# haampie/Homogenization.jl

Measured on AMD Instinct MI355X. Metric: fine-DOF updates/sec per V-cycle (3D Tet64), higher is better.
Workload: dtype f64; 1 GPU; 3D Tet64 checkerboard, 32^3 unit cubes x 6 tets, refinements=5 (BASELINE config 3); cells=196608, nf=6545, levels=6, smoothing_steps=3, smoothing_steps_coarse=2, coarse_solver=device CG, Chebyshev(4)-of-Jacobi preconditioner, rtol 1e-13, spare_vector_bytes=10294394880, lazy_top_form=2

## Files before the change

homogenization.jl_amd/csrc/hmg_context.cpp:

```cpp
#include "../../include/hmg.h"
#include "hmg_objects.hpp"

#include <algorithm>

namespace hmg {

std::recursive_mutex &lifetime_mutex()
{
    static std::recursive_mutex m;
    return m;
}

std::atomic<int64_t> &device_allocs()
{
    static std::atomic<int64_t> n{0};
    return n;
}

namespace {

void vec_pool_trim(hmg_ctx *c)
{
    LifetimeLock lock(lifetime_mutex());
    if (c->vec_pool.empty()) return;
// ... 206 lines not shown
}

int64_t hmg_ctx_counter(hmg_ctx *ctx, const char *name)
{
    if (!ctx || !name) return -1;
    const std::string n(name);
    if (n == "wave_launches") return ctx->wave_launches;
    if (n == "slab2_launches") return ctx->slab2_launches;
    if (n == "rows_launches") return ctx->rows_launches;
    if (n == "small_launches") return ctx->small_launches;
    if (n == "comm_calls") return ctx->comm_calls;
    if (n == "device_allocs") return device_allocs().load();
    if (n == "spare_bytes") return ctx->spare_bytes;
    if (n == "fcg_bytes") return ctx->fcg_bytes;
    if (n == "lazy_top_form") return ctx->last_top_form;
    if (n == "comm_nranks") return ctx->comm ? ctx->comm_nranks : 0;
    return -1;
}

int hmg_ctx_release_memory(hmg_ctx *ctx)
{
    HMG_TRY
    need(ctx != nullptr, "null ctx");
    vec_pool_trim(ctx);
    HMG_END
}

int hmg_ctx_set_option(hmg_ctx *ctx, const char *name, int64_t value)
{
    HMG_TRY
    need(ctx && name, "null argument");
    std::string n(name);
    static const std::pair<const char *, bool hmg_ctx::*> flags[] = {
        {"coarse_probe", &hmg_ctx::coarse_probe}, {"fuse_cg", &hmg_ctx::fuse_cg_default}, {"fold_x", &hmg_ctx::fold_x},
        {"swap_rp", &hmg_ctx::swap_rp}, {"fold_prolong", &hmg_ctx::fold_prolong}, {"zero_entry", &hmg_ctx::zero_entry},
        {"fold_restrict", &hmg_ctx::fold_restrict}, {"lazy_dead", &hmg_ctx::lazy_dead}, {"fold_faces", &hmg_ctx::fold_faces},
        {"lean_post", &hmg_ctx::lean_post}, {"lazy_post", &hmg_ctx::lazy_post}, {"prolong_in_image", &hmg_ctx::prolong_in_image},
        {"comm_rehearsal", &hmg_ctx::comm_rehearsal}};
    for (const auto &f : flags)
        if (n == f.first) {
            ctx->*f.second = value != 0;
            return 0;
        }
    if (n == "apply_threads")
        ctx->L.apply_threads = (int)value;
    else if (n == "apply_wg512")
        ctx->L.apply_wg512 = value != 0;
    else if (n == "apply_pack")
        ctx->L.apply_pack = value != 0;
    else if (n == "apply_small")
        ctx->L.apply_small = value != 0;
// ... 172 lines not shown
```

homogenization.jl_amd/csrc/hmg_device.hpp:

```cpp
#pragma once
#include <hip/hip_runtime.h>

#include <cstdint>

namespace hmg {

constexpr int TABLE_PAD = 3 * 1024;

__host__ __device__ inline int rows_slot(int m, int i, int j, int nei, int off_int, int &cls)
{
    if (j == 0) {
        cls = i == 0 ? 4 : i == m ? 5 : 1;
        return i == 0 ? 0 : i == m ? 1 : 3 + i - 1;
    }
    if (i == 0) {
        cls = j == m ? 6 : 2;
        return j == m ? 2 : 3 + nei + j - 1;
    }
    if (i + j == m) {
        cls = 3;
        return 3 + 2 * nei + j - 1;
    }
    cls = 0;
    return off_int + (j - 1) * (m - 1) - (((j - 1) * j) >> 1) + i - 1;
// ... 79 lines not shown
    int nclasses;
    double wc_lambda;
    double *blockpart;
    SlabTables slab;
};

struct ApplyArgs {
    double alpha, lambda;
    const double *x;
    const double *x2;
    double *xout;
    double *xacc;
    int a_num, a_den;
    const double *x3;
    int c_num, c_den;
    const double *xcoarse;
    int64_t ldc;
    const double *src;
    double *out;
    double *rcoarse;
    int64_t ldrc;
    const double *scal;
    int s_num, s_den;
    double *blockpart;
    const uint8_t *mult;
    int flags;
    int64_t ncells_prefix;
    int64_t out_ld;
    const int32_t *cell_list;
    int64_t ncell_list;
    int64_t nwork;
    const int32_t *cell_class;
// ... 28 lines not shown
    int apply_wave;
    int64_t wave_grid;
    int64_t *n_wave_launches;
    int apply_slab2;
    int64_t *n_slab2_launches;
    int64_t slab2_grid;
    int restrict_slab2;
    int slab2_force;
    int64_t *n_rows_launches;
};

void launch_apply(const Launch &L, const LevelDev &lv, const MeshDev &mesh, double alpha, double lambda,
                  const double *x, const double *src, double *out, int use_mask);
size_t apply_lds_bytes(const LevelDev &lv);
bool apply_restricts(const Launch &L, const LevelDev &lv);
void launch_apply_fused_kernel(const Launch &L, const LevelDev &lv, const MeshDev &mesh, ApplyArgs a);
void launch_apply_fused_reduce(const Launch &L, const MeshDev &mesh, int slot_pap, int slot_rr);
void launch_apply_args(const Launch &L, const LevelDev &lv, const MeshDev &mesh, ApplyArgs a);
bool apply_wave_ok(const Launch &L, const LevelDev &lv, const MeshDev &mesh, const ApplyArgs &a, bool fused);
void launch_apply_wave(const Launch &L, const LevelDev &lv, const MeshDev &mesh, const ApplyArgs &a, bool fused);
bool apply_slab2_ok(const Launch &L, const LevelDev &lv, const MeshDev &mesh, const ApplyArgs &a);
void launch_apply_slab2(const Launch &L, const LevelDev &lv, const MeshDev &mesh, const ApplyArgs &a, bool fused);
void launch_apply_rows(const Launch &L, const LevelDev &lv, const MeshDev &mesh, const ApplyArgs &a, bool fused, bool wd);
void launch_prolong_add_wide(const Launch &L, const LevelDev &fine, const LevelDev &coarse, int64_t ncells, const double *xc,
                             double *xf);
int64_t launch_norm2_unique_wide(const Launch &L, const LevelDev &lv, const MeshDev &mesh, const double *x);
bool apply_small_ok(const Launch &L, const LevelDev &lv, const MeshDev &mesh, const ApplyArgs &a, bool fused);
void launch_apply_small(const Launch &L, const LevelDev &lv, const MeshDev &mesh, const ApplyArgs &a, bool fused);
void launch_weight_cache(const Launch &L, const LevelDev &lv, const double *coef_rep, int nclasses, double lambda, double *wcache);

// ... 76 lines not shown
```

homogenization.jl_amd/csrc/hmg_kernels.hip:

```cpp
#include "hmg_device.hpp"
#include "hmg_stencil.hpp"

#include <cstdio>
#include <stdexcept>
#include <string>

namespace hmg {

__global__ void __launch_bounds__(256) k_finalize(const double *__restrict__ partials, int n, double *scal, int slot)
{
    __shared__ double red[4];
    double v = 0.0;
    for (int i = threadIdx.x; i < n; i += 256) v += partials[i];
    double s = block_sum(v, red);
    if (threadIdx.x == 0) scal[slot] = s;
}

#ifdef HMG_PHASE_TIMING
#define HMG_STAMP(i)                                                                     \
    do {    \
        if (a.blockpart && !a.cell_list && tid == 0)                                     \
            a.blockpart[2 * (size_t)a.nwork + 8 * cell + (i)] = (double)wall_clock64(); \
    } while (0)
#define HMG_SLAB_T0() const long long _t0 = wall_clock64(); long long _tl = _t0; double _ph[5] = {0, 0, 0, 0, 0}
// ... 174 lines not shown
            if (wave == NW - 1) {
                const int cbase = (1 + lv.nface + lv.nedge) * NDIR;
                for (int idx = cbase + lane; idx < lv.ncls * NDIR; idx += 64) {
                    double w = 0.0;
#pragma unroll
                    for (int t = 0; t < NTERM; ++t) w += lv.ctab[(size_t)idx * NTERM + t] * sc7[t];
                    W[idx - cbase] = w;
                }
            }
        }
        if (FUSED) {
#pragma unroll
            for (int q = 0; q < 4; ++q) mq[q] = a.mult ? __builtin_amdgcn_readfirstlane(mqr[q]) : 0x01010101u;
        }
    };
    constexpr bool rows_late = WC && LF == 2;
    constexpr bool WEARLY = false;
    if (EARLY && !rows_late) issue_rows();
    if (WEARLY) issue_words();
    const double *xc = a.x + cell * lv.ld;
    double rr = 0.0, pap = 0.0;
    {
        const double *x2c = FUSED && a.x2 ? a.x2 + cell * lv.ld : nullptr;
        double *xoc = FUSED && a.xout ? a.xout + cell * lv.ld : nullptr;
        double *xac = FUSED && a.xacc ? a.xacc + cell * lv.ld : nullptr;
        const double *x3c = FUSED && a.x3 ? a.x3 + cell * lv.ld : nullptr;
        const double beta = x2c ? a.scal[a.s_num] / a.scal[a.s_den] : 0.0;
        const double ax = xac || x3c ? a.scal[a.a_num] / a.scal[a.a_den] : 0.0;
        const double c2 = x3c ? a.scal[a.c_num] / a.scal[a.c_den] : 0.0;
        const double *ccol = FUSED && !RS && a.xcoarse ? a.xcoarse + cell * a.ldc : nullptr;
        constexpr bool cgather = FUSED && CG;
        double *cs = xs + nf + lv.lds_g1;
        double cval = 0.0;
        if (ccol && !cgather) {
            if (tid < lv.nf_coarse) cval = ccol[tid];
            for (int q = tid + NT; q < lv.nf_coarse; q += NT) cs[q] = ccol[q];
        }
        auto prolong = [&](double v, uint32_t w) {
            const uint32_t pa = w & 0xffffu, pb = w >> 16;
            if (pa == pb) return v + cs[pa];
            v += 0.5 * cs[pa];
            return v + 0.5 * cs[pb];
        };
        if (cgather && ccol) {
            constexpr int NC = 2;
            double cv2[NC];
            int cl2[NC];
#pragma unroll
            for (int q = 0; q < NC; ++q) {
                const int c = tid + q * NT;
                if (c < lv.nf_coarse) {
                    cv2[q] = ccol[c];
                    cl2[q] = lv.clpos[c];
                }
            }
            double xv[SPT];
            uint64_t pw[SPT];
#pragma unroll
            for (int q = 0; q < SPT; ++q) {
                const int t = tid + q * NT;
                if (t < nf) {
                    xv[q] = xc[t];
                    pw[q] = lv.par64[t];
                }
            }
            if (EARLY) finish_tables();
#pragma unroll
            for (int q = 0; q < NC; ++q)
                if (tid + q * NT < lv.nf_coarse) xs[cl2[q]] = cv2[q];
// ... 63 lines not shown
                }
            }
            if (EARLY && rows_late) issue_rows();
            if (EARLY) finish_tables();
#pragma unroll
            for (int q = 0; q < SPT; ++q) {
                const int t = tid + q * NT;
                if (t < nf) {
                    const double v = axpy1(beta, x2v[q], xv[q]);
                    if (LF == 2 && xoc) xoc[t] = v;
                    rr += v * v;
                    xs[lp[q]] = v;
                }
            }
        }
        constexpr int HB = FUSED ? (SPT + 1) / 2 : SPT;
        const bool xzero = FUSED && (RS || RB == 0) && (a.flags & 128);
        if (!light && !light2 && !(cgather && ccol)) {
#pragma unroll
        for (int q0 = 0; q0 < SPT; q0 += HB) {
            double xv[HB], x2v[HB], xav[HB];
            int lp[HB];
            uint32_t pw[HB];
#pragma unroll
            for (int q = 0; q < HB; ++q) {
                const int t = tid + (q0 + q) * NT;
                if (q0 + q < SPT && t < nf) {
                    xv[q] = xzero ? 0.0 : xc[t];
                    x2v[q] = x2c ? x2c[t] : 0.0;
                    xav[q] = xac ? xac[t] : x3c ? x3c[t] : 0.0;
                    lp[q] = lv.lpos[t];
                    if (FUSED && !cgather) pw[q] = ccol ? lv.par32[t] : 0u;
                }
            }
            if (EARLY && q0 == 0) finish_tables();
            if (FUSED && q0 == 0 && ccol && !cgather) {
                if (tid < lv.nf_coarse) cs[tid] = cval;
                __syncthreads();
            }
#pragma unroll
            for (int q = 0; q < HB; ++q) {
                const int t = tid + (q0 + q) * NT;
                if (q0 + q < SPT && t < nf) {
                    double v = xv[q];
                    if (FUSED) {
                        if (!cgather && ccol) v = prolong(v, pw[q]);
                        if (xac) xac[t] = axpy1(ax, x2v[q], xav[q]);
                        if (x3c) {
                            const double t1 = axpy1(ax, x2v[q], v);
                            const double p2 = axpy1(beta, x2v[q], xav[q]);
                            v = axpy1(c2, p2, t1);
                        } else if (x2c)
                            v = axpy1(beta, x2v[q], v);
                        if (xoc) xoc[t] = v;
                        if (!RS) rr += v * v;
                    }
                    xs[lp[q]] = v;
                }
            }
        }
        }
        for (int t = tid + SPT * NT; t < nf; t += NT) {
            double v = xzero ? 0.0 : xc[t];
            if (FUSED) {
                const double pv = x2c ? x2c[t] : 0.0;
                if (!cgather && ccol) v = prolong(v, lv.par32[t]);
                if (xac) xac[t] = axpy1(ax, pv, xac[t]);
                if (x3c) {
                    const double t1 = axpy1(ax, pv, v);
                    const double p2 = axpy1(beta, pv, x3c[t]);
                    v = axpy1(c2, p2, t1);
                } else if (x2c)
                    v = axpy1(beta, pv, v);
                if (xoc) xoc[t] = v;
                rr += v * v;
            }
            xs[lv.lpos[t]] = v;
        }
    }

    HMG_STAMP(1);
    __builtin_amdgcn_sched_barrier(0);
    if (!WEARLY) issue_words();
// ... 463 lines not shown
size_t apply_lds_bytes(const LevelDev &lv)
{
    return sizeof(double) * (size_t)(WSZ + lv.lds_g0 + lv.nf + lv.lds_g1);
}

bool apply_restricts(const Launch &L, const LevelDev &lv)
{
    if (!(lv.dim == 3 && apply_lds_bytes(lv) <= 160 * 1024 && L.apply_threads == 0 && lv.rs_word &&
          lv.rs_w && lv.nf_coarse > 0 && lv.nei <= 64 && lv.nedge == 6 && lv.ncorner == 4))
        return false;
    if (lv.nf > 2048)
        return lv.blk_R == 6 && lv.nblk <= 960 && L.apply_wg512 && lv.nfi <= 512;
    return lv.nf > 192 && lv.nf <= 1024 && lv.blk_R == 4 && lv.nblk <= 192 && lv.nfi <= 128 && lv.rs_lp != nullptr;
}

static size_t apply_lds_bytes_rb(const LevelDev &lv)
{
    return sizeof(double) * (size_t)(WSZ_RB + lv.lds_g0 + lv.nf + lv.lds_g1);
}

template <bool FUSED>
static void check_apply_bases(const ApplyArgs &a, const MeshDev &mesh)
{
    if (!a.x) throw std::runtime_error("operator apply: null input vector");
    if (!FUSED && !a.out) throw std::runtime_error("operator apply: a plain launch needs an output vector");
    if (a.rcoarse && a.ldrc <= 0) throw std::runtime_error("operator apply: epilogue restriction without the coarse column stride");
    if (FUSED && (!a.blockpart || !a.scal)) throw std::runtime_error("operator apply: fused launch without its reduction scratch");
    if (!mesh.coef) throw std::runtime_error("operator apply: no operator coefficients on the device (hmg_grid_set_operator)");
    if ((a.flags & 1) && !mesh.dmask) throw std::runtime_error("operator apply: constraint requested without a Dirichlet mask");
    if (a.xcoarse && !a.xout) throw std::runtime_error("operator apply: folded prolongation without xout");
    if ((a.flags & 128) && !(FUSED && a.x3 && a.x2 && a.xout && !a.xcoarse))
        throw std::runtime_error("operator apply: the zero-input form exists for the residual with two pending x-updates only");
}

static bool weight_cache_ok(const Launch &L, const LevelDev &lv, const MeshDev &mesh, const ApplyArgs &a)
{
    return L.weight_cache && lv.wcache && mesh.cell_class && lv.dim == 3 && lv.ncls == 15 && !(a.flags & (2 | 8 | 16)) &&
           (a.alpha == 1.0 || a.alpha == -1.0) && a.lambda == mesh.wc_lambda;
}

template <int DIM, int NT, int SPT, bool FUSED, int RB = 0, bool WD = false, bool CG = false, bool RS = false, bool WC = false, int LF = 0>
static void launch_apply_generic(const Launch &L, const LevelDev &lv, const MeshDev &mesh, const ApplyArgs &a, size_t lds)
{
    auto kern = k_apply<DIM, NT, SPT, FUSED, RB, WD, CG, RS, WC, LF>;
    if (a.rcoarse && !RS) throw std::runtime_error("operator apply: this instantiation cannot restrict in its epilogue");
    if ((a.flags & 128) && !(FUSED && (RS || RB == 0)))
        throw std::runtime_error("operator apply: this instantiation cannot take a zero input that is not in memory");
    if (FUSED && a.xcoarse && !CG) lds += sizeof(double) * (size_t)lv.nf_coarse;
    if (lds > 48 * 1024)
        HMG_HIP_CHECK(hipFuncSetAttribute((const void *)kern, hipFuncAttributeMaxDynamicSharedMemorySize, (int)lds));
    const int64_t nblocks = a.cell_list ? a.ncell_list : a.ncells_prefix ? a.ncells_prefix : mesh.ncells;
    if (nblocks == 0) return;
    check_apply_bases<FUSED>(a, mesh);
    ApplyArgs b = a;
    b.nwork = nblocks;
    b.cell_class = WC ? mesh.cell_class : nullptr;
    if (WC && !weight_cache_ok(L, lv, mesh, a)) throw std::runtime_error("operator apply: class-weight cache not usable for this launch");
    if (L.cell_order && RB && !a.cell_list && !a.ncells_prefix && mesh.cell_perm) {
        b.cell_list = mesh.cell_perm;
        b.ncell_list = nblocks;
    }
    const int64_t grid = NT == 64 ? std::min<int64_t>(nblocks, 32 * (int64_t)L.num_cu) : nblocks;
    hipLaunchKernelGGL(kern, dim3((unsigned)grid), dim3(NT), lds, L.stream, lv, mesh.coef, mesh.dmask, b);
    check_launch();
}

template <int DIM, bool FUSED, bool WD = false>
static void launch_apply_dim(const Launch &L, const LevelDev &lv, const MeshDev &mesh, const ApplyArgs &a)
{
    const size_t lds = apply_lds_bytes(lv);
    if constexpr (DIM == 3 && !WD) {
        if (apply_wave_ok(L, lv, mesh, a, FUSED)) {
            launch_apply_wave(L, lv, mesh, a, FUSED);
            return;
        }
        if (apply_small_ok(L, lv, mesh, a, FUSED)) {
            launch_apply_small(L, lv, mesh, a, FUSED);
            return;
        }
    }
    const bool force_slab2 = DIM == 3 && !WD && L.slab2_force && mesh.slab.head && mesh.slab.nslab >= 2 && lv.nf > 2048 &&
                             !a.xcoarse && !a.rcoarse && !(a.flags & (4 | 8));
    if (DIM == 2 && lds > 160 * 1024) {
        launch_apply_rows(L, lv, mesh, a, FUSED, WD);
        return;
// ... 67 lines not shown
                    launch_apply_generic<DIM, 512, 13, FUSED, DIM == 3 ? 6 : 0>(L, lv, mesh, a, apply_lds_bytes_rb(lv));
                else
                    launch_apply_generic<DIM, 512, 13, FUSED>(L, lv, mesh, a, lds);
            } else
                launch_apply_generic<DIM, 640, 11, FUSED>(L, lv, mesh, a, lds);
        }
    } else if (DIM == 3 && lv.blk_R == 6 && lv.nblk <= 960 && lv.nei <= 64 && lv.nedge == 6 && lv.ncorner == 4) {
        if constexpr (!WD) {
            if (L.apply_wg512 && lv.nfi <= 512) {
                const bool cg = FUSED && DIM == 3 && a.xcoarse && (a.flags & 64) && lv.par64 && lv.clpos && !a.x2 && !a.xacc && !a.x3 &&
                                lv.nf <= 13 * 512 && lv.nf_coarse <= 2 * 512;
                const bool rs = !cg && FUSED && DIM == 3 && a.rcoarse && lv.rs_word && lv.rs_w && !a.xcoarse;
                constexpr int R6 = DIM == 3 ? 6 : 0;
                constexpr bool F3 = FUSED && DIM == 3;
                if (DIM == 3 && weight_cache_ok(L, lv, mesh, a)) {
                    if (cg)
                        launch_apply_generic<DIM, 512, 13, FUSED, R6, false, F3, false, DIM == 3>(L, lv, mesh, a, apply_lds_bytes_rb(lv));
                    else if (rs)
                        launch_apply_generic<DIM, 512, 13, FUSED, R6, false, false, F3, DIM == 3>(L, lv, mesh, a, apply_lds_bytes_rb(lv));
                    else if (FUSED && !a.x2 && !a.xacc && !a.x3 && !a.xcoarse && !a.rcoarse)
                        launch_apply_generic<DIM, 512, 13, FUSED, R6, false, false, false, DIM == 3, F3 ? 1 : 0>(L, lv, mesh, a, apply_lds_bytes_rb(lv));
                    else if (FUSED && a.x2 && (!a.xout || a.xout != a.x2) && !a.xacc && !a.x3 && !a.xcoarse && !a.rcoarse)
                        launch_apply_generic<DIM, 512, 13, FUSED, R6, false, false, false, DIM == 3, F3 ? 2 : 0>(L, lv, mesh, a, apply_lds_bytes_rb(lv));
                    else
                        launch_apply_generic<DIM, 512, 13, FUSED, R6, false, false, false, DIM == 3>(L, lv, mesh, a, apply_lds_bytes_rb(lv));
                    return;
                }
                if (cg)
                    launch_apply_generic<DIM, 512, 13, FUSED, R6, false, F3>(L, lv, mesh, a, apply_lds_bytes_rb(lv));
                else if (rs)
                    launch_apply_generic<DIM, 512, 13, FUSED, R6, false, false, F3>(L, lv, mesh, a, apply_lds_bytes_rb(lv));
                else
                    launch_apply_generic<DIM, 512, 13, FUSED, R6>(L, lv, mesh, a, apply_lds_bytes_rb(lv));
                return;
            }
        }
        launch_apply_generic<DIM, 1024, 7, FUSED, DIM == 3 ? 6 : 0, WD>(L, lv, mesh, a, apply_lds_bytes_rb(lv));
    }
    else
        launch_apply_generic<DIM, 1024, 7, FUSED, 0, WD>(L, lv, mesh, a, lds);
}

void launch_apply(const Launch &L, const LevelDev &lv, const MeshDev &mesh, double alpha, double lambda,
                  const double *x, const double *src, double *out, int use_mask)
// ... 1412 lines not shown
```

homogenization.jl_amd/csrc/hmg_objects.hpp:

```cpp
#pragma once

#include "../../include/hmg.h"
#include "hmg_device.hpp"
#include "hmg_host.hpp"

#include <atomic>
#include <memory>
#include <mutex>
#include <stdexcept>
#include <string>
#include <vector>

struct ncclComm;

using namespace hmg;

#define HIPCHK(expr)                                                                            \
    do {                                                                                        \
        hipError_t _e = (expr);                                                                 \
        if (_e != hipSuccess)                                                                   \
            throw std::runtime_error(std::string("HIP error: ") + hipGetErrorString(_e) + " (" #expr ")"); \
    } while (0)

namespace hmg {
// ... 119 lines not shown
    bool pending = false;
    int budget = 0;
    int generation = 0;
};

}

struct hmg_ctx {
    int refs = 1;
    ApplyTimer timer;
    bool fuse_cg_default = true;
    bool fold_x = true;
    bool swap_rp = true;
    bool fold_prolong = true;
    bool lazy_dead = true;
    bool fold_faces = true;
    bool lean_post = true;
    bool lazy_post = true;
    int lazy_top = 2;
    bool zero_entry = true;
    bool fold_restrict = true;
    bool prolong_in_image = true;
    int device = 0;
    hipStream_t stream = nullptr;
    bool own_stream = false;
    DevBuf<double> partials, scal, rpart;
    Launch L{};
    int coarse_maxit = 5000;
    int coarse_check = 25;
    bool coarse_probe = true;
    double coarse_rtol = 1e-13;
    int coarse_poly = 4;
    double coarse_poly_ratio = 20.0;
    ncclComm *comm = nullptr;
    int comm_nranks = 1, comm_rank = 0;
    hipStream_t comm_stream = nullptr;
    hipEvent_t ev_packed = nullptr, ev_summed = nullptr;
    int64_t comm_calls = 0, comm_doubles = 0;
    int64_t small_launches = 0;
    int64_t wave_launches = 0;
    int64_t slab2_launches = 0;
    int64_t rows_launches = 0;
    int64_t spare_bytes = 0;
    int64_t fcg_bytes = 0;
    int last_top_form = 0;
    bool vec_pool_on = true;
    std::vector<std::pair<size_t, void *>> vec_pool;
    bool comm_rehearsal = false;
    int64_t overlap_min_doubles = 524288;
    std::vector<struct hmg_grid *> probe_grids;
};

struct hmg_grid {
    int refs = 1;
    hmg_ctx *ctx = nullptr;
    int dim = 0, nlevels = 0;
    std::vector<LevelTables> lt;
    std::vector<std::unique_ptr<LevelBufs>> lb;
    std::vector<LevelDev> ld;
// ... 148 lines not shown
```

homogenization.jl_amd/csrc/hmg_smooth.cpp:

```cpp
#include "../../include/hmg.h"
#include "hmg_objects.hpp"

#include <algorithm>
#include <cmath>

namespace hmg {

void set_slab(hmg_grid *g, const LevelDev &lv)
{
    const LevelBufs &B = *g->lb[lv.level - 1];
    g->md.slab.head = B.slab_head.p;
    g->md.slab.ld_word = B.slab_ld_word.p;
    g->md.slab.cp_word = B.slab_cp_word.p;
    g->md.slab.cp_slot = B.slab_cp_slot.p;
    g->md.slab.nslab = B.nslab;
    g->md.slab.lds_nodes = B.slab_lds_nodes;
    g->md.slab.max_surf = B.slab_max_surf;
    g->md.slab.max_int = B.slab_max_int;
}

namespace {

struct TimedRegion {
    hmg_ctx *c;
// ... 94 lines not shown
        HIPCHK(hipMemcpyAsync(lead, d, sizeof(lead), hipMemcpyDeviceToHost, c->stream));
        HIPCHK(hipStreamSynchronize(c->stream));
        for (int k = 0; k < 3; ++k) g->cut_agreed[k] = (int64_t)std::llround(lead[k]);
    }
    g->cut_agreed_ready = true;
}

void apply_then_sum(hmg_grid *g, const LevelDev &lv, ApplyArgs a, bool fused, int slot_pap, int slot_rr,
                    bool sum_out = true, bool faces = true)
{
    hmg_ctx *c = g->ctx;
    const Launch &L = c->L;
    set_slab(g, lv);
    ensure_weight_cache(g);
    const double streams = ((a.flags & 128) ? 0.0 : 1.0) + (a.out ? 1.0 : 0.0) + (a.src ? 1.0 : 0.0) + (a.x2 ? 1.0 : 0.0) + (a.xout ? 1.0 : 0.0) +
                           (a.xacc ? 2.0 : 0.0) + (a.x3 ? 1.0 : 0.0) + (a.xcoarse ? (double)lv.nf_coarse / (double)lv.nf : 0.0) +
                           (a.rcoarse ? (double)lv.nf_coarse / (double)lv.nf : 0.0);
    TimedRegion tr(g, lv, 8.0 * (double)lv.nf * (double)g->md.ncells * streams);
    if (has_exchange(g) && g->part) agree_on_cut(g);
    const bool has_cut = has_exchange(g) && g->part && g->cut_agreed[0] >= 0 &&
                         g->cut_agreed[0] + g->cut_agreed[1] + g->cut_agreed[2] > 0;
    const int64_t global_cut = has_cut ? g->cut_agreed[0] * lv.nfi + g->cut_agreed[1] * lv.nei + g->cut_agreed[2] : 0;
    const bool overlap = has_cut && (g->sharers ? g->p2p_begin != nullptr : g->ex_begin != nullptr) && g->ex_end && g->overlap &&
                         global_cut >= std::max<int64_t>(1, c->overlap_min_doubles);
    auto launch = [&](const int32_t *list, int64_t n) {
        ApplyArgs b = a;
        b.cell_list = list;
        b.ncell_list = n;
        if (fused)
            launch_apply_fused_kernel(L, lv, g->md, b);
        else
            launch_apply_args(L, lv, g->md, b);
// ... 50 lines not shown
enum class Role {
    Plain,
    Pre,
    PostTop,
    PostBelow,
};

enum class Tail {
    Full,
    ScratchP,
    Top2,
    Top3,
    DeadXp,
    DeadDefer,
    DeadDefer2,
    DeadX2,
};

struct SmoothForm {
    bool swap_rp = false;
    bool ride = false;
    Tail tail = Tail::Full;
    bool x_zero = false;
};

struct DeferredX {
    int rs = -1;
    int pap = S_PAP;
    bool two_updates = false;
    int a_num = -1, a_den = -1, b_num = -1, b_den = -1;
};

SmoothForm smooth_form(const hmg_grid *g, int level, int steps, Role role)
{
    const LevelDev &lv = lev(g, level);
    const hmg_ctx *c = g->ctx;
    const bool lean = c->lean_post && (role == Role::PostTop || role == Role::PostBelow);
    const bool dead = role == Role::Pre || (lean && role == Role::PostBelow);
    SmoothForm f;
    if (!g->fuse_cg) {
        f.tail = dead ? Tail::DeadXp : lean ? Tail::ScratchP : Tail::Full;
        return f;
    }
    const bool faces = c->fold_faces && lv.dim == 3 && lv.nfi > 0;
    f.swap_rp = role != Role::Plain && c->swap_rp && steps > 0;
    f.ride = faces;
    if (role == Role::Pre && c->fold_x)
        f.tail = steps >= 2 && c->lazy_dead ? Tail::DeadDefer2 : Tail::DeadDefer;
    else if (dead)
        f.tail = steps >= 2 && c->lazy_post ? Tail::DeadX2 : Tail::DeadXp;
    else if (lean && steps >= 2 && c->lazy_top > 0 && faces)
        f.tail = steps >= 3 && c->lazy_top > 1 && g->top_spare.n >= (size_t)lv.ld * (size_t)g->md.ncells ? Tail::Top3 : Tail::Top2;
    else if (lean)
        f.tail = Tail::ScratchP;
    return f;
}

}

bool reserve_top_spare(hmg_grid *g, bool must)
{
    hmg_ctx *c = g->ctx;
    const LevelDev &lv = g->ld[(size_t)g->nlevels - 1];
// ... 24 lines not shown
    if (g->ctx) {
        if (g->top_spare.p) (void)hipStreamSynchronize(g->ctx->stream);
        g->ctx->spare_bytes -= (int64_t)(g->top_spare.n * sizeof(double));
    }
    g->top_spare.release();
}

bool wants_top_spare(const hmg_grid *g, int level)
{
    return g->ctx && g->ctx->lazy_top > 1 && level == g->nlevels && g->dim == 3 && g->ld[(size_t)level - 1].nfi > 0;
}

namespace {

DeferredX smooth(hmg_grid *g, int level, int steps, hmg_vec *x, hmg_vec *b, hmg_vec *r, hmg_vec *p, hmg_vec *Ap,
                 const SmoothForm &f, const hmg_vec *xcoarse = nullptr)
{
    const LevelDev &lv = lev(g, level);
    const Launch &L = g->ctx->L;
    const int64_t n = vec_len(x);
    {
        ApplyArgs a{};
        a.alpha = -1.0;
        a.lambda = g->lambda;
        a.x = x->d;
        a.src = b->d;
        a.out = r->d;
        a.flags = 1;
        if (f.x_zero) {
            need(!xcoarse, "zero initial guess with a coarse-grid correction");
            launch_copy(L, r->d, b->d, n);
            launch_mask(L, lv, g->md, r->d, 0);
            interface_sum(g, lv, r->d);
        } else if (xcoarse) {
            a.xcoarse = xcoarse->d;
            a.ldc = lev(g, level - 1).ld;
            a.xout = x->d;
            if (g->ctx->prolong_in_image && apply_lds_bytes(lv) > 48 * 1024) a.flags |= 64;
            apply_then_sum(g, lv, a, true, -1, -1);
        } else {
            apply_then_sum(g, lv, a, false, -1, -1);
        }
    }
    int cur = S_RS, other = S_RS2;
    if (!g->fuse_cg || steps <= 0) {
        launch_copy_dot(L, p->d, r->d, n, cur);
        scalar_sum(g, cur, 1);
        for (int i = 0; i < steps; ++i) {
            apply(g, lv, 1.0, p->d, nullptr, Ap->d, 1);
            interface_sum(g, lv, Ap->d);
            launch_dot(L, p->d, Ap->d, n, S_PAP);
            scalar_sum(g, S_PAP, 1);
            const bool last = i == steps - 1;
// ... 35 lines not shown
        apply_then_sum(g, lv, args(i), true, S_PAP, i == 0 ? cur : -1, true, !ride);
        const double *r_in = r->d;
        if (i == 0 && f.swap_rp) {
            exchange_rp();
            r_in = p->d;
        }
        if (ride)
            launch_cg_rupdate_faces(L, lv, g->md, r_in, r->d, Ap->d, n, cur, S_PAP, other);
        else
            launch_cg_rupdate(L, r_in, r->d, Ap->d, n, cur, S_PAP, other);
        scalar_sum(g, other, 1);
        std::swap(cur, other);
    };
    const int last = steps - 1;
    for (int i = 0; i < last; ++i) {
        if (f.tail == Tail::Top3 && i == last - 1) {
            ApplyArgs a = args(i);
            a.xout = g->top_spare.p;
            a.xacc = nullptr;
            apply_then_sum(g, lv, a, true, S_PAP2, -1, true, false);
            launch_cg_rupdate_faces(L, lv, g->md, r->d, r->d, Ap->d, n, cur, S_PAP2, S_RS3);
            scalar_sum(g, S_RS3, 1);
            continue;
        }
        step(i, f.ride);
    }
    if (f.tail == Tail::Top2 || f.tail == Tail::Top3) g->ctx->last_top_form = f.tail == Tail::Top3 ? 2 : 1;
    ApplyArgs a = args(last);
    switch (f.tail) {
    case Tail::Full:
    case Tail::ScratchP:
        step(last, f.ride && f.tail == Tail::ScratchP);
        launch_cg_xp_update(L, x->d, p->d, r->d, n, other, S_PAP, cur, other, f.tail == Tail::Full ? 1 : 0);
        return {};
    case Tail::DeadXp:
    case Tail::DeadDefer:
        a.out = nullptr;
        apply_then_sum(g, lv, a, true, S_PAP, last == 0 ? cur : -1, true, true);
        if (last == 0 && f.swap_rp) exchange_rp();
        if (f.tail == Tail::DeadDefer) return DeferredX{cur};
        launch_cg_xp_update(L, x->d, p->d, r->d, n, cur, S_PAP, cur, other, 0);
        return {};
    case Tail::DeadDefer2:
    case Tail::DeadX2:
        a.out = a.xout = a.xacc = nullptr;
        apply_then_sum(g, lv, a, true, S_PAP2, -1);
        if (f.tail == Tail::DeadX2) {
            launch_cg_x2_update(L, x->d, p->d, r->d, n, other, S_PAP, cur, other, cur, S_PAP2);
            return {};
        }
        return DeferredX{cur, S_PAP2, true, other, S_PAP, cur, other};
    case Tail::Top2:
        a.xout = a.xacc = nullptr;
        apply_then_sum(g, lv, a, true, S_PAP2, -1, true, false);
        launch_cg_rupdate_faces_x(L, lv, g->md, r->d, r->d, Ap->d, n, cur, S_PAP2, other, x->d, p->d, other, S_PAP, cur, other,
                                  nullptr, 0, 0);
        scalar_sum(g, other, 1);
        return {};
    case Tail::Top3:
        a.x2 = g->top_spare.p;
        a.xout = a.xacc = nullptr;
        a.s_num = S_RS3;
        a.s_den = cur;
        apply_then_sum(g, lv, a, true, S_PAP3, -1, true, false);
        launch_cg_rupdate_faces_x(L, lv, g->md, r->d, r->d, Ap->d, n, S_RS3, S_PAP3, other, x->d, g->top_spare.p, cur, S_PAP2,
                                  S_RS3, cur, p->d, other, S_PAP);
// ... 1 lines not shown
        return {};
    }
    return {};
}

bool zero_entry_ok(const hmg_grid *g, int k, int steps)
{
    if (!g->ctx->zero_entry) return false;
    if (k == 1) return true;
    if (steps != 2 || smooth_form(g, k, steps, Role::Pre).tail != Tail::DeadDefer2) return false;
    const LevelDev &lv = g->ld[k - 1];
    if (lv.blk_R > 0) return g->ctx->fold_restrict && apply_restricts(g->ctx->L, lv);
    return true;
}

void vcycle_down(hmg_grid *g, int k, int steps, hmg_vec **st, bool inside = false, bool x_zero = false, int steps_next = -1)
{
    hmg_vec **cur = st + 5 * (k - 1);
    hmg_vec **nxt = st + 5 * (k - 2);
    const Launch &L = g->ctx->L;
    SmoothForm form = smooth_form(g, k, steps, Role::Pre);
    need(!x_zero || form.tail == Tail::DeadDefer2, "zero initial guess: the pre-smoother does not defer both x-updates");
    form.x_zero = x_zero;
    const DeferredX dx = smooth(g, k, steps, cur[0], cur[1], cur[2], cur[3], cur[4], form);
    const bool skip_fill = inside && steps_next >= 0 && zero_entry_ok(g, k - 1, steps_next);
    if (dx.rs >= 0) {
        ApplyArgs a{};
        a.alpha = -1.0;
        a.lambda = g->lambda;
        a.x = cur[0]->d;
        a.x2 = cur[3]->d;
        a.xout = cur[0]->d;
        if (dx.two_updates) {
            a.x3 = cur[2]->d;
            a.a_num = dx.a_num;
            a.a_den = dx.a_den;
            a.s_num = dx.b_num;
            a.s_den = dx.b_den;
            a.c_num = dx.rs;
            a.c_den = dx.pap;
        } else {
            a.s_num = dx.rs;
            a.s_den = dx.pap;
        }
        a.src = cur[1]->d;
        a.out = cur[2]->d;
        a.flags = 1 | (x_zero ? 128 : 0);
        if (g->ctx->fold_restrict && apply_restricts(L, lev(g, k))) {
            if (inside) a.out = nullptr;
            a.rcoarse = nxt[1]->d;
            a.ldrc = lev(g, k - 1).ld;
            apply_then_sum(g, lev(g, k), a, true, -1, -1, false);
            if (!skip_fill) launch_fill(L, nxt[0]->d, vec_len(nxt[0]), 0.0);
            return;
        }
        apply_then_sum(g, lev(g, k), a, true, -1, -1, false);
    } else {
        apply(g, lev(g, k), -1.0, cur[0]->d, cur[1]->d, cur[2]->d, 1);
    }
    restrict_level(g, k, cur[2]->d, nxt[1]->d);
    if (!skip_fill) launch_fill(L, nxt[0]->d, vec_len(nxt[0]), 0.0);
}

void vcycle_up(hmg_grid *g, int k, int steps, hmg_vec **st, Role role)
{
    hmg_vec **cur = st + 5 * (k - 1);
    hmg_vec **nxt = st + 5 * (k - 2);
    const Launch &L = g->ctx->L;
    const bool fold_p = g->ctx->fold_prolong && g->fuse_cg && apply_lds_bytes(lev(g, k)) <= 160 * 1024 &&
                        apply_lds_bytes(lev(g, k)) + sizeof(double) * (size_t)lev(g, k - 1).nf <= 80 * 1024;
    if (!fold_p) launch_prolong_add(L, lev(g, k), lev(g, k - 1), g->md.ncells, nxt[0]->d, cur[0]->d);
    smooth(g, k, steps, cur[0], cur[1], cur[2], cur[3], cur[4], smooth_form(g, k, steps, role), fold_p ? nxt[0] : nullptr);
}

}

void vcycle(hmg_grid *g, int k, int steps, int steps_coarse, hmg_vec **st, bool top, bool zero_guess)
{
    if (k == 1) {
        hmg_vec **cur = st;
        coarse_solve(g, cur[1], cur[0]);
        return;
    }
    const bool x_zero = (zero_guess || !top) && zero_entry_ok(g, k, steps);
    if (top && zero_guess && !x_zero) launch_fill(g->ctx->L, st[5 * (k - 1)]->d, vec_len(st[5 * (k - 1)]), 0.0);
    vcycle_down(g, k, steps, st, true, x_zero, steps_coarse);
    vcycle(g, k - 1, steps_coarse, steps_coarse, st, false);
    if (top) g->ctx->last_top_form = 0;
    vcycle_up(g, k, steps, st, top ? Role::PostTop : Role::PostBelow);
}

}

extern "C" {

int hmg_grid_reserve_spare(hmg_grid *g, int enable)
{
    HMG_TRY
    need(g != nullptr, "null grid");
    need(g->ctx != nullptr, "this grid was created without a device context (host tables only)");
    if (enable) {
        (void)reserve_top_spare(g, true);
    } else {
        release_top_spare(g);
// ... 66 lines not shown
            double *d = c->L.scal + S_HOST;
            HIPCHK(hipMemcpyAsync(d, &failed, sizeof(double), hipMemcpyHostToDevice, c->stream));
            scalar_sum(g, S_HOST, 1);
            HIPCHK(hipMemcpyAsync(&failed, d, sizeof(double), hipMemcpyDeviceToHost, c->stream));
            HIPCHK(hipStreamSynchronize(c->stream));
            if (failed > 0.0 && local_failure.empty())
                local_failure = "placement tuning: another rank could not set it up (nothing was changed on this rank)";
        }
        if (!local_failure.empty()) throw std::runtime_error(local_failure);
        const int nb = (int)blk.size();
        auto run = [&](const std::vector<int> &a) {
            assign(a);
            launch_fill(c->L, state[0]->d, n, 0.5);
            launch_fill(c->L, state[1]->d, n, 1.0);
            HIPCHK(hipEventRecord(e0, c->stream));
            vcycle_down(g, level, steps, states, true, false, 2);
            vcycle_up(g, level, steps, states, Role::PostTop);
            HIPCHK(hipEventRecord(e1, c->stream));
            HIPCHK(hipEventSynchronize(e1));
            float ms = 0.f;
            HIPCHK(hipEventElapsedTime(&ms, e0, e1));
            return (double)ms;
        };
        (void)run(first);
        uint64_t rng = 0x9E3779B97F4A7C15ull;
        auto next = [&]() {
            rng ^= rng << 13;
            rng ^= rng >> 7;
            rng ^= rng << 17;
            return rng;
        };
        t_best = 1e300;
// ... 46 lines not shown
    HMG_END
}

static void check_two_levels(hmg_grid *g, int level, hmg_vec **states)
{
    need(g && g->has_op && states, "null argument or operator not set");
    need(level >= 2 && level <= g->nlevels, "level out of range (2..nlevels)");
    for (int l = level - 1; l <= level; ++l)
        for (int q = 0; q < 5; ++q) check_vec(g, l, states[5 * (l - 1) + q], "states[]");
}

int hmg_vcycle_down(hmg_grid *g, int level, int steps, hmg_vec **states)
{
    HMG_TRY
    check_two_levels(g, level, states);
    vcycle_down(g, level, steps, states);
    HMG_END
}

int hmg_vcycle_up(hmg_grid *g, int level, int steps, hmg_vec **states)
{
    HMG_TRY
    check_two_levels(g, level, states);
    vcycle_up(g, level, steps, states, Role::PostTop);
    HMG_END
}

}
```

Baseline: 11.18 billion fine-DOF updates/s.

## Defer third pre-smoother x-update and fold coarse post-smoother x-update into prolongation

Adds a DeadDefer3 pre-smoother tail that keeps a third pending x-update (x4) and applies it inside the fused residual/restrict kernel instead of a separate update pass. It also lets the coarse level's post-smoother skip its final x2 update and hand the pending p/r updates up, where the fine-level fused prolongation kernel finishes the coarse x on the fly. Both changes aim to remove full-vector read/write passes and kernel launches per V-cycle. The cost is extra streams read inside the kernels, more template instantiations, and tighter eligibility conditions.

```diff
diff --git a/homogenization.jl_amd/csrc/hmg_context.cpp b/homogenization.jl_amd/csrc/hmg_context.cpp
--- a/homogenization.jl_amd/csrc/hmg_context.cpp
+++ b/homogenization.jl_amd/csrc/hmg_context.cpp
@@ -244,6 +244,8 @@
     if (n == "spare_bytes") return ctx->spare_bytes;
     if (n == "fcg_bytes") return ctx->fcg_bytes;
     if (n == "lazy_top_form") return ctx->last_top_form;
+    if (n == "lazy_pre_form") return ctx->last_pre_form;
+    if (n == "coarse_x_folds") return ctx->coarse_x_folds;
     if (n == "comm_nranks") return ctx->comm ? ctx->comm_nranks : 0;
     return -1;
 }
@@ -264,7 +266,7 @@
     static const std::pair<const char *, bool hmg_ctx::*> flags[] = {
         {"coarse_probe", &hmg_ctx::coarse_probe}, {"fuse_cg", &hmg_ctx::fuse_cg_default}, {"fold_x", &hmg_ctx::fold_x},
         {"swap_rp", &hmg_ctx::swap_rp}, {"fold_prolong", &hmg_ctx::fold_prolong}, {"zero_entry", &hmg_ctx::zero_entry},
-        {"fold_restrict", &hmg_ctx::fold_restrict}, {"lazy_dead", &hmg_ctx::lazy_dead}, {"fold_faces", &hmg_ctx::fold_faces},
+        {"fold_restrict", &hmg_ctx::fold_restrict}, {"lazy_dead", &hmg_ctx::lazy_dead}, {"lazy_pre", &hmg_ctx::lazy_pre}, {"fold_coarse_x", &hmg_ctx::fold_coarse_x}, {"fold_faces", &hmg_ctx::fold_faces},
         {"lean_post", &hmg_ctx::lean_post}, {"lazy_post", &hmg_ctx::lazy_post}, {"prolong_in_image", &hmg_ctx::prolong_in_image},
         {"comm_rehearsal", &hmg_ctx::comm_rehearsal}};
     for (const auto &f : flags)
diff --git a/homogenization.jl_amd/csrc/hmg_device.hpp b/homogenization.jl_amd/csrc/hmg_device.hpp
--- a/homogenization.jl_amd/csrc/hmg_device.hpp
+++ b/homogenization.jl_amd/csrc/hmg_device.hpp
@@ -117,8 +117,11 @@
     int a_num, a_den;
     const double *x3;
     int c_num, c_den;
+    const double *x4;
+    int d_num, d_den;
     const double *xcoarse;
     int64_t ldc;
+    const double *xc_p, *xc_r;
     const double *src;
     double *out;
     double *rcoarse;
@@ -177,6 +180,8 @@
                   const double *x, const double *src, double *out, int use_mask);
 size_t apply_lds_bytes(const LevelDev &lv);
 bool apply_restricts(const Launch &L, const LevelDev &lv);
+bool apply_folds_coarse_x(const Launch &L, const LevelDev &lv);
+bool apply_defers3(const Launch &L, const LevelDev &lv);
 void launch_apply_fused_kernel(const Launch &L, const LevelDev &lv, const MeshDev &mesh, ApplyArgs a);
 void launch_apply_fused_reduce(const Launch &L, const MeshDev &mesh, int slot_pap, int slot_rr);
 void launch_apply_args(const Launch &L, const LevelDev &lv, const MeshDev &mesh, ApplyArgs a);
diff --git a/homogenization.jl_amd/csrc/hmg_kernels.hip b/homogenization.jl_amd/csrc/hmg_kernels.hip
--- a/homogenization.jl_amd/csrc/hmg_kernels.hip
+++ b/homogenization.jl_amd/csrc/hmg_kernels.hip
@@ -212,7 +212,7 @@
             for (int q = 0; q < 4; ++q) mq[q] = a.mult ? __builtin_amdgcn_readfirstlane(mqr[q]) : 0x01010101u;
         }
     };
-    constexpr bool rows_late = WC && LF == 2;
+    constexpr bool rows_late = WC && (LF == 2 || LF == 5);
     constexpr bool WEARLY = false;
     if (EARLY && !rows_late) issue_rows();
     if (WEARLY) issue_words();
@@ -226,6 +226,9 @@
         const double beta = x2c ? a.scal[a.s_num] / a.scal[a.s_den] : 0.0;
         const double ax = xac || x3c ? a.scal[a.a_num] / a.scal[a.a_den] : 0.0;
         const double c2 = x3c ? a.scal[a.c_num] / a.scal[a.c_den] : 0.0;
+        constexpr bool X4 = FUSED && RS && LF == 4;
+        const double *x4c = X4 && a.x4 ? a.x4 + cell * lv.ld : nullptr;
+        const double dx4 = x4c ? a.scal[a.d_num] / a.scal[a.d_den] : 0.0;
         const double *ccol = FUSED && !RS && a.xcoarse ? a.xcoarse + cell * a.ldc : nullptr;
         constexpr bool cgather = FUSED && CG;
         double *cs = xs + nf + lv.lds_g1;
@@ -242,15 +245,31 @@
         };
         if (cgather && ccol) {
             constexpr int NC = 2;
-            double cv2[NC];
+            constexpr bool CX = cgather && LF == 5;
+            const double *cpc = CX ? a.xc_p + cell * a.ldc : nullptr, *crc = CX ? a.xc_r + cell * a.ldc : nullptr;
+            const double cxa = CX ? to_sgpr(a.scal[a.a_num] / a.scal[a.a_den]) : 0.0;
+            const double cxb = CX ? to_sgpr(a.scal[a.s_num] / a.scal[a.s_den]) : 0.0;
+            const double cxc = CX ? to_sgpr(a.scal[a.c_num] / a.scal[a.c_den]) : 0.0;
+            double cv2[NC], cp2[CX ? NC : 1], cr2[CX ? NC : 1];
             int cl2[NC];
 #pragma unroll
             for (int q = 0; q < NC; ++q) {
                 const int c = tid + q * NT;
                 if (c < lv.nf_coarse) {
                     cv2[q] = ccol[c];
+                    if (CX) {
+                        cp2[q] = cpc[c];
+                        cr2[q] = crc[c];
+                    }
                     cl2[q] = lv.clpos[c];
                 }
+            }
+            if (CX) {
+#pragma unroll
+                for (int q = 0; q < NC; ++q)
+                    if (tid + q * NT < lv.nf_coarse) cv2[q] = axpy1(cxc, axpy1(cxb, cp2[q], cr2[q]), axpy1(cxa, cp2[q], cv2[q]));
+                __builtin_amdgcn_sched_barrier(0);
+                if (EARLY && rows_late) issue_rows();
             }
             double xv[SPT];
             uint64_t pw[SPT];
@@ -344,12 +363,12 @@
                 }
             }
         }
-        constexpr int HB = FUSED ? (SPT + 1) / 2 : SPT;
+        constexpr int HB = X4 ? (SPT + 2) / 3 : FUSED ? (SPT + 1) / 2 : SPT;
         const bool xzero = FUSED && (RS || RB == 0) && (a.flags & 128);
         if (!light && !light2 && !(cgather && ccol)) {
 #pragma unroll
         for (int q0 = 0; q0 < SPT; q0 += HB) {
-            double xv[HB], x2v[HB], xav[HB];
+            double xv[HB], x2v[HB], xav[HB], x4v[X4 ? HB : 1];
             int lp[HB];
             uint32_t pw[HB];
 #pragma unroll
@@ -357,6 +376,7 @@
                 const int t = tid + (q0 + q) * NT;
                 if (q0 + q < SPT && t < nf) {
                     xv[q] = xzero ? 0.0 : xc[t];
+                    if (X4) x4v[q] = x4c ? x4c[t] : 0.0;
                     x2v[q] = x2c ? x2c[t] : 0.0;
                     xav[q] = xac ? xac[t] : x3c ? x3c[t] : 0.0;
                     lp[q] = lv.lpos[t];
@@ -377,6 +397,7 @@
                         if (!cgather && ccol) v = prolong(v, pw[q]);
                         if (xac) xac[t] = axpy1(ax, x2v[q], xav[q]);
                         if (x3c) {
+                            if (X4 && x4c) v = axpy1(dx4, x4v[q], v);
                             const double t1 = axpy1(ax, x2v[q], v);
                             const double p2 = axpy1(beta, x2v[q], xav[q]);
                             v = axpy1(c2, p2, t1);
@@ -397,6 +418,7 @@
                 if (!cgather && ccol) v = prolong(v, lv.par32[t]);
                 if (xac) xac[t] = axpy1(ax, pv, xac[t]);
                 if (x3c) {
+                    if (X4 && x4c) v = axpy1(dx4, x4c[t], v);
                     const double t1 = axpy1(ax, pv, v);
                     const double p2 = axpy1(beta, pv, x3c[t]);
                     v = axpy1(c2, p2, t1);
@@ -890,6 +912,18 @@
     return lv.nf > 192 && lv.nf <= 1024 && lv.blk_R == 4 && lv.nblk <= 192 && lv.nfi <= 128 && lv.rs_lp != nullptr;
 }
 
+bool apply_defers3(const Launch &L, const LevelDev &lv)
+{
+    return apply_restricts(L, lv) && lv.nf > 2048 && lv.nf <= 13 * 512;
+}
+
+bool apply_folds_coarse_x(const Launch &L, const LevelDev &lv)
+{
+    return lv.dim == 3 && apply_lds_bytes(lv) <= 160 * 1024 && L.apply_threads == 0 && L.apply_wg512 && lv.blk_R == 6 && lv.nblk <= 960 &&
+           lv.nei <= 64 && lv.nedge == 6 && lv.ncorner == 4 && lv.nfi <= 512 && lv.par64 && lv.clpos && lv.nf > 2048 &&
+           lv.nf <= 13 * 512 && lv.nf_coarse > 0 && lv.nf_coarse <= 2 * 512;
+}
+
 static size_t apply_lds_bytes_rb(const LevelDev &lv)
 {
     return sizeof(double) * (size_t)(WSZ_RB + lv.lds_g0 + lv.nf + lv.lds_g1);
@@ -920,6 +954,8 @@
 {
     auto kern = k_apply<DIM, NT, SPT, FUSED, RB, WD, CG, RS, WC, LF>;
     if (a.rcoarse && !RS) throw std::runtime_error("operator apply: this instantiation cannot restrict in its epilogue");
+    if (a.xc_p && !(CG && LF == 5)) throw std::runtime_error("operator apply: this instantiation cannot finish the coarse x");
+    if (a.x4 && LF != 4) throw std::runtime_error("operator apply: this instantiation cannot carry a third pending x-update");
     if ((a.flags & 128) && !(FUSED && (RS || RB == 0)))
         throw std::runtime_error("operator apply: this instantiation cannot take a zero input that is not in memory");
     if (FUSED && a.xcoarse && !CG) lds += sizeof(double) * (size_t)lv.nf_coarse;
@@ -945,6 +981,12 @@
 static void launch_apply_dim(const Launch &L, const LevelDev &lv, const MeshDev &mesh, const ApplyArgs &a)
 {
     const size_t lds = apply_lds_bytes(lv);
+    if (a.x4 && !(FUSED && DIM == 3 && !WD && a.x3 && a.x2 && a.xout && a.rcoarse && !a.xcoarse && !a.xacc && !(a.flags & 128) &&
+                  apply_defers3(L, lv)))
+        throw std::runtime_error("operator apply: a third pending x-update (x4) where no kernel carries it");
+    if ((a.xc_p || a.xc_r) && !(FUSED && DIM == 3 && !WD && a.xc_p && a.xc_r && a.xcoarse && (a.flags & 64) && !a.x2 && !a.xacc && !a.x3 &&
+                                !a.rcoarse && apply_folds_coarse_x(L, lv)))
+        throw std::runtime_error("operator apply: pending coarse x-updates (xc_p, xc_r) where no kernel carries them");
     if constexpr (DIM == 3 && !WD) {
         if (apply_wave_ok(L, lv, mesh, a, FUSED)) {
             launch_apply_wave(L, lv, mesh, a, FUSED);
@@ -1042,8 +1084,12 @@
                 constexpr int R6 = DIM == 3 ? 6 : 0;
                 constexpr bool F3 = FUSED && DIM == 3;
                 if (DIM == 3 && weight_cache_ok(L, lv, mesh, a)) {
-                    if (cg)
+                    if (cg && a.xc_p)
+                        launch_apply_generic<DIM, 512, 13, FUSED, R6, false, F3, false, DIM == 3, F3 ? 5 : 0>(L, lv, mesh, a, apply_lds_bytes_rb(lv));
+                    else if (cg)
                         launch_apply_generic<DIM, 512, 13, FUSED, R6, false, F3, false, DIM == 3>(L, lv, mesh, a, apply_lds_bytes_rb(lv));
+                    else if (rs && a.x4)
+                        launch_apply_generic<DIM, 512, 13, FUSED, R6, false, false, F3, DIM == 3, F3 ? 4 : 0>(L, lv, mesh, a, apply_lds_bytes_rb(lv));
                     else if (rs)
                         launch_apply_generic<DIM, 512, 13, FUSED, R6, false, false, F3, DIM == 3>(L, lv, mesh, a, apply_lds_bytes_rb(lv));
                     else if (FUSED && !a.x2 && !a.xacc && !a.x3 && !a.xcoarse && !a.rcoarse)
@@ -1054,8 +1100,12 @@
                         launch_apply_generic<DIM, 512, 13, FUSED, R6, false, false, false, DIM == 3>(L, lv, mesh, a, apply_lds_bytes_rb(lv));
                     return;
                 }
-                if (cg)
+                if (cg && a.xc_p)
+                    launch_apply_generic<DIM, 512, 13, FUSED, R6, false, F3, false, false, F3 ? 5 : 0>(L, lv, mesh, a, apply_lds_bytes_rb(lv));
+                else if (cg)
                     launch_apply_generic<DIM, 512, 13, FUSED, R6, false, F3>(L, lv, mesh, a, apply_lds_bytes_rb(lv));
+                else if (rs && a.x4)
+                    launch_apply_generic<DIM, 512, 13, FUSED, R6, false, false, F3, false, F3 ? 4 : 0>(L, lv, mesh, a, apply_lds_bytes_rb(lv));
                 else if (rs)
                     launch_apply_generic<DIM, 512, 13, FUSED, R6, false, false, F3>(L, lv, mesh, a, apply_lds_bytes_rb(lv));
                 else
diff --git a/homogenization.jl_amd/csrc/hmg_objects.hpp b/homogenization.jl_amd/csrc/hmg_objects.hpp
--- a/homogenization.jl_amd/csrc/hmg_objects.hpp
+++ b/homogenization.jl_amd/csrc/hmg_objects.hpp
@@ -157,9 +157,11 @@
     bool swap_rp = true;
     bool fold_prolong = true;
     bool lazy_dead = true;
+    bool lazy_pre = true;
     bool fold_faces = true;
     bool lean_post = true;
     bool lazy_post = true;
+    bool fold_coarse_x = true;
     int lazy_top = 2;
     bool zero_entry = true;
     bool fold_restrict = true;
@@ -186,6 +188,8 @@
     int64_t rows_launches = 0;
     int64_t spare_bytes = 0;
     int64_t fcg_bytes = 0;
+    int64_t coarse_x_folds = 0;
+    int last_pre_form = 0;
     int last_top_form = 0;
     bool vec_pool_on = true;
     std::vector<std::pair<size_t, void *>> vec_pool;
diff --git a/homogenization.jl_amd/csrc/hmg_smooth.cpp b/homogenization.jl_amd/csrc/hmg_smooth.cpp
--- a/homogenization.jl_amd/csrc/hmg_smooth.cpp
+++ b/homogenization.jl_amd/csrc/hmg_smooth.cpp
@@ -132,8 +132,8 @@
     set_slab(g, lv);
     ensure_weight_cache(g);
     const double streams = ((a.flags & 128) ? 0.0 : 1.0) + (a.out ? 1.0 : 0.0) + (a.src ? 1.0 : 0.0) + (a.x2 ? 1.0 : 0.0) + (a.xout ? 1.0 : 0.0) +
-                           (a.xacc ? 2.0 : 0.0) + (a.x3 ? 1.0 : 0.0) + (a.xcoarse ? (double)lv.nf_coarse / (double)lv.nf : 0.0) +
-                           (a.rcoarse ? (double)lv.nf_coarse / (double)lv.nf : 0.0);
+                           (a.xacc ? 2.0 : 0.0) + (a.x3 ? 1.0 : 0.0) + (a.x4 ? 1.0 : 0.0) + (a.xcoarse ? (double)lv.nf_coarse / (double)lv.nf : 0.0) +
+                           (a.rcoarse ? (double)lv.nf_coarse / (double)lv.nf : 0.0) + (a.xc_p ? 2.0 * (double)lv.nf_coarse / (double)lv.nf : 0.0);
     TimedRegion tr(g, lv, 8.0 * (double)lv.nf * (double)g->md.ncells * streams);
     if (has_exchange(g) && g->part) agree_on_cut(g);
     const bool has_cut = has_exchange(g) && g->part && g->cut_agreed[0] >= 0 &&
@@ -214,6 +214,7 @@
     DeadXp,
     DeadDefer,
     DeadDefer2,
+    DeadDefer3,
     DeadX2,
 };
 
@@ -221,6 +222,7 @@
     bool swap_rp = false;
     bool ride = false;
     Tail tail = Tail::Full;
+    bool hand_up = false;
     bool x_zero = false;
 };
 
@@ -229,6 +231,9 @@
     int pap = S_PAP;
     bool two_updates = false;
     int a_num = -1, a_den = -1, b_num = -1, b_den = -1;
+    bool three_updates = false;
+    int d_num = -1, d_den = -1;
+    const double *p = nullptr, *r = nullptr;
 };
 
 SmoothForm smooth_form(const hmg_grid *g, int level, int steps, Role role)
@@ -245,8 +250,12 @@
     const bool faces = c->fold_faces && lv.dim == 3 && lv.nfi > 0;
     f.swap_rp = role != Role::Plain && c->swap_rp && steps > 0;
     f.ride = faces;
-    if (role == Role::Pre && c->fold_x)
+    if (role == Role::Pre && c->fold_x) {
         f.tail = steps >= 2 && c->lazy_dead ? Tail::DeadDefer2 : Tail::DeadDefer;
+        if (f.tail == Tail::DeadDefer2 && steps >= 3 && c->lazy_pre && faces && c->fold_restrict && apply_defers3(c->L, lv) &&
+            g->top_spare.n >= (size_t)lv.ld * (size_t)g->md.ncells)
+            f.tail = Tail::DeadDefer3;
+    }
     else if (dead)
         f.tail = steps >= 2 && c->lazy_post ? Tail::DeadX2 : Tail::DeadXp;
     else if (lean && steps >= 2 && c->lazy_top > 0 && faces)
@@ -301,7 +310,7 @@
 namespace {
 
 DeferredX smooth(hmg_grid *g, int level, int steps, hmg_vec *x, hmg_vec *b, hmg_vec *r, hmg_vec *p, hmg_vec *Ap,
-                 const SmoothForm &f, const hmg_vec *xcoarse = nullptr)
+                 const SmoothForm &f, const hmg_vec *xcoarse = nullptr, const DeferredX *cx = nullptr)
 {
     const LevelDev &lv = lev(g, level);
     const Launch &L = g->ctx->L;
@@ -324,6 +333,18 @@
             a.ldc = lev(g, level - 1).ld;
             a.xout = x->d;
             if (g->ctx->prolong_in_image && apply_lds_bytes(lv) > 48 * 1024) a.flags |= 64;
+            if (cx && cx->rs >= 0) {
+                need(cx->two_updates && cx->p && cx->r && (a.flags & 64), "pending coarse x-updates where the residual cannot carry them");
+                a.xc_p = cx->p;
+                a.xc_r = cx->r;
+                a.a_num = cx->a_num;
+                a.a_den = cx->a_den;
+                a.s_num = cx->b_num;
+                a.s_den = cx->b_den;
+                a.c_num = cx->rs;
+                a.c_den = cx->pap;
+                g->ctx->coarse_x_folds += 1;
+            }
             apply_then_sum(g, lv, a, true, -1, -1);
         } else {
             apply_then_sum(g, lv, a, false, -1, -1);
@@ -389,7 +410,7 @@
     };
     const int last = steps - 1;
     for (int i = 0; i < last; ++i) {
-        if (f.tail == Tail::Top3 && i == last - 1) {
+        if ((f.tail == Tail::Top3 || f.tail == Tail::DeadDefer3) && i == last - 1) {
             ApplyArgs a = args(i);
             a.xout = g->top_spare.p;
             a.xacc = nullptr;
@@ -420,11 +441,30 @@
     case Tail::DeadX2:
         a.out = a.xout = a.xacc = nullptr;
         apply_then_sum(g, lv, a, true, S_PAP2, -1);
+        if (f.tail == Tail::DeadX2 && f.hand_up) {
+            DeferredX d{cur, S_PAP2, true, other, S_PAP, cur, other};
+            d.p = p->d;
+            d.r = r->d;
+            return d;
+        }
         if (f.tail == Tail::DeadX2) {
             launch_cg_x2_update(L, x->d, p->d, r->d, n, other, S_PAP, cur, other, cur, S_PAP2);
             return {};
         }
         return DeferredX{cur, S_PAP2, true, other, S_PAP, cur, other};
+    case Tail::DeadDefer3:
+        a.x2 = g->top_spare.p;
+        a.out = a.xout = a.xacc = nullptr;
+        a.s_num = S_RS3;
+        a.s_den = cur;
+        apply_then_sum(g, lv, a, true, S_PAP3, -1);
+        {
+            DeferredX d{S_RS3, S_PAP3, true, cur, S_PAP2, S_RS3, cur};
+            d.three_updates = true;
+            d.d_num = other;
+            d.d_den = S_PAP;
+            return d;
+        }
     case Tail::Top2:
         a.xout = a.xacc = nullptr;
         apply_then_sum(g, lv, a, true, S_PAP2, -1, true, false);
@@ -456,7 +496,7 @@
     return true;
 }
 
-void vcycle_down(hmg_grid *g, int k, int steps, hmg_vec **st, bool inside = false, bool x_zero = false, int steps_next = -1)
+int vcycle_down(hmg_grid *g, int k, int steps, hmg_vec **st, bool inside = false, bool x_zero = false, int steps_next = -1)
 {
     hmg_vec **cur = st + 5 * (k - 1);
     hmg_vec **nxt = st + 5 * (k - 2);
@@ -465,14 +505,21 @@
     need(!x_zero || form.tail == Tail::DeadDefer2, "zero initial guess: the pre-smoother does not defer both x-updates");
     form.x_zero = x_zero;
     const DeferredX dx = smooth(g, k, steps, cur[0], cur[1], cur[2], cur[3], cur[4], form);
+    const int deferred = dx.rs < 0 ? 0 : dx.three_updates ? 3 : dx.two_updates ? 2 : 1;
     const bool skip_fill = inside && steps_next >= 0 && zero_entry_ok(g, k - 1, steps_next);
     if (dx.rs >= 0) {
         ApplyArgs a{};
         a.alpha = -1.0;
         a.lambda = g->lambda;
         a.x = cur[0]->d;
-        a.x2 = cur[3]->d;
+        a.x2 = dx.three_updates ? g->top_spare.p : cur[3]->d;
         a.xout = cur[0]->d;
+        if (dx.three_updates) {
+            need(g->ctx->fold_restrict && apply_defers3(L, lev(g, k)), "three pending x-updates where the local residual cannot carry them");
+            a.x4 = cur[3]->d;
+            a.d_num = dx.d_num;
+            a.d_den = dx.d_den;
+        }
         if (dx.two_updates) {
             a.x3 = cur[2]->d;
             a.a_num = dx.a_num;
@@ -494,7 +541,7 @@
             a.ldrc = lev(g, k - 1).ld;
             apply_then_sum(g, lev(g, k), a, true, -1, -1, false);
             if (!skip_fill) launch_fill(L, nxt[0]->d, vec_len(nxt[0]), 0.0);
-            return;
+            return deferred;
         }
         apply_then_sum(g, lev(g, k), a, true, -1, -1, false);
     } else {
@@ -502,34 +549,55 @@
     }
     restrict_level(g, k, cur[2]->d, nxt[1]->d);
     if (!skip_fill) launch_fill(L, nxt[0]->d, vec_len(nxt[0]), 0.0);
-}
-
-void vcycle_up(hmg_grid *g, int k, int steps, hmg_vec **st, Role role)
+    return deferred;
+}
+
+DeferredX vcycle_up(hmg_grid *g, int k, int steps, hmg_vec **st, Role role, const DeferredX *cx = nullptr, bool hand_up = false)
 {
     hmg_vec **cur = st + 5 * (k - 1);
     hmg_vec **nxt = st + 5 * (k - 2);
     const Launch &L = g->ctx->L;
     const bool fold_p = g->ctx->fold_prolong && g->fuse_cg && apply_lds_bytes(lev(g, k)) <= 160 * 1024 &&
                         apply_lds_bytes(lev(g, k)) + sizeof(double) * (size_t)lev(g, k - 1).nf <= 80 * 1024;
+    need(!(cx && cx->rs >= 0) || fold_p, "pending coarse x-updates without the folded prolongation");
     if (!fold_p) launch_prolong_add(L, lev(g, k), lev(g, k - 1), g->md.ncells, nxt[0]->d, cur[0]->d);
-    smooth(g, k, steps, cur[0], cur[1], cur[2], cur[3], cur[4], smooth_form(g, k, steps, role), fold_p ? nxt[0] : nullptr);
-}
-
-}
-
-void vcycle(hmg_grid *g, int k, int steps, int steps_coarse, hmg_vec **st, bool top, bool zero_guess)
+    SmoothForm form = smooth_form(g, k, steps, role);
+    form.hand_up = hand_up && form.tail == Tail::DeadX2;
+    return smooth(g, k, steps, cur[0], cur[1], cur[2], cur[3], cur[4], form, fold_p ? nxt[0] : nullptr, cx);
+}
+
+bool coarse_x_folds(const hmg_grid *g, int k, int steps_below)
+{
+    const hmg_ctx *c = g->ctx;
+    if (k < 3 || !c->fold_coarse_x || !c->lazy_post || !c->fold_prolong || !c->lean_post || !g->fuse_cg || !c->prolong_in_image) return false;
+    const LevelDev &lv = g->ld[(size_t)k - 1];
+    if (!(apply_lds_bytes(lv) > 48 * 1024 && apply_lds_bytes(lv) <= 160 * 1024 &&
+          apply_lds_bytes(lv) + sizeof(double) * (size_t)g->ld[(size_t)k - 2].nf <= 80 * 1024))
+        return false;
+    return apply_folds_coarse_x(c->L, lv) && smooth_form(g, k - 1, steps_below, Role::PostBelow).tail == Tail::DeadX2;
+}
+
+DeferredX vcycle_level(hmg_grid *g, int k, int steps, int steps_coarse, hmg_vec **st, bool top, bool zero_guess, bool hand_up)
 {
     if (k == 1) {
         hmg_vec **cur = st;
         coarse_solve(g, cur[1], cur[0]);
-        return;
+        return {};
     }
     const bool x_zero = (zero_guess || !top) && zero_entry_ok(g, k, steps);
     if (top && zero_guess && !x_zero) launch_fill(g->ctx->L, st[5 * (k - 1)]->d, vec_len(st[5 * (k - 1)]), 0.0);
-    vcycle_down(g, k, steps, st, true, x_zero, steps_coarse);
-    vcycle(g, k - 1, steps_coarse, steps_coarse, st, false);
+    const int deferred = vcycle_down(g, k, steps, st, true, x_zero, steps_coarse);
+    if (top) g->ctx->last_pre_form = deferred;
+    const DeferredX cx = vcycle_level(g, k - 1, steps_coarse, steps_coarse, st, false, false, coarse_x_folds(g, k, steps_coarse));
     if (top) g->ctx->last_top_form = 0;
-    vcycle_up(g, k, steps, st, top ? Role::PostTop : Role::PostBelow);
+    return vcycle_up(g, k, steps, st, top ? Role::PostTop : Role::PostBelow, &cx, hand_up);
+}
+
+}
+
+void vcycle(hmg_grid *g, int k, int steps, int steps_coarse, hmg_vec **st, bool top, bool zero_guess)
+{
+    (void)vcycle_level(g, k, steps, steps_coarse, st, top, zero_guess, false);
 }
 
 }
@@ -626,8 +694,8 @@
             launch_fill(c->L, state[0]->d, n, 0.5);
             launch_fill(c->L, state[1]->d, n, 1.0);
             HIPCHK(hipEventRecord(e0, c->stream));
-            vcycle_down(g, level, steps, states, true, false, 2);
-            vcycle_up(g, level, steps, states, Role::PostTop);
+            (void)vcycle_down(g, level, steps, states, true, false, 2);
+            (void)vcycle_up(g, level, steps, states, Role::PostTop);
             HIPCHK(hipEventRecord(e1, c->stream));
             HIPCHK(hipEventSynchronize(e1));
             float ms = 0.f;
@@ -704,7 +772,7 @@
 {
     HMG_TRY
     check_two_levels(g, level, states);
-    vcycle_down(g, level, steps, states);
+    g->ctx->last_pre_form = vcycle_down(g, level, steps, states);
     HMG_END
 }
 
@@ -712,7 +780,7 @@
 {
     HMG_TRY
     check_two_levels(g, level, states);
-    vcycle_up(g, level, steps, states, Role::PostTop);
+    (void)vcycle_up(g, level, steps, states, Role::PostTop);
     HMG_END
 }
 
```

Result: faster. 11.36 billion fine-DOF updates/s, median of 6 (+1.6%).
